# davidfang00/opticalflowdiffusion

Measured on AMD Instinct MI355X. Metric: UNet denoise steps/sec @ 2x436x1024 flow, bs=16, higher is better.
Workload: dtype bf16

## Files before the change

opticalflowdiffusion_amd/csrc/la_fused.hip:

```cpp
#include <cstdlib>
#include <type_traits>
#include "blocks.h"
#include "la_common.h"

namespace ofd {

template <int C>
struct XRaw {
    u32x4 v[C / 16];
};

template <int C>
__device__ __forceinline__ void load_raw_x(const bf16_t* __restrict__ xrow, XRaw<C>& r, int half) {
#pragma unroll
    for (int s = 0; s < C / 16; ++s) r.v[s] = *(const u32x4*)(xrow + 16 * s + 8 * half);
}

template <int N16, class At>
__device__ __forceinline__ void la_stage(unsigned char* dst, const bf16_t* __restrict__ src, int tid, At at) {
    static_assert(N16 % (8 * 256) == 0, "whole turns of eight units per thread");
    for (int i0 = tid; i0 < N16; i0 += 8 * 256) {
        uint4 v[8];
#pragma unroll
        for (int k = 0; k < 8; ++k) v[k] = ((const uint4*)src)[at(i0 + k * 256)];
#pragma unroll
        for (int k = 0; k < 8; ++k) ((uint4*)dst)[i0 + k * 256] = v[k];
    }
}
template <int N16>
__device__ __forceinline__ void la_stage(unsigned char* dst, const bf16_t* __restrict__ src, int tid) {
    la_stage<N16>(dst, src, tid, [](int i) { return i; });
}

typedef __bf16 la_bf16x2 __attribute__((ext_vector_type(2)));
template <int C>
__device__ __forceinline__ void norm_stats(const XRaw<C>& r, float eps, float& rstd, float& off) {
    const la_bf16x2 one = __builtin_bit_cast(la_bf16x2, 0x3f803f80u);
    float s1 = 0.0f, s2 = 0.0f;
#pragma unroll
    for (int s = 0; s < C / 16; ++s)
#pragma unroll
        for (int j = 0; j < 4; ++j) {
            const la_bf16x2 w = __builtin_bit_cast(la_bf16x2, (uint32_t)r.v[s][j]);
            s1 = __builtin_amdgcn_fdot2_f32_bf16(w, one, s1, false);
            s2 = __builtin_amdgcn_fdot2_f32_bf16(w, w, s2, false);
        }
    s1 += __shfl_xor(s1, 32, 64);
    s2 += __shfl_xor(s2, 32, 64);
    const float mean = s1 * (1.0f / C);
    const float var = fmaxf(__builtin_fmaf(-mean, mean, s2 * (1.0f / C)), 0.0f);
    rstd = rsqrtf(var + eps);
    off = -mean * rstd;
}
template <int C>
__device__ __forceinline__ void norm_x(const XRaw<C>& r, float eps, bf16x8 (&xs)[C / 16]) {
    float rstd, off;
    norm_stats<C>(r, eps, rstd, off);
#pragma unroll
    for (int s = 0; s < C / 16; ++s)
#pragma unroll
        for (int j = 0; j < 4; ++j) {
            const uint32_t w = r.v[s][j];
            xs[s][2 * j] = (__bf16)__builtin_fmaf(bf2f((bf16_t)(w & 0xffffu)), rstd, off);
            xs[s][2 * j + 1] = (__bf16)__builtin_fmaf(bf2f((bf16_t)(w >> 16)), rstd, off);
        }
}

template <int C>
__device__ __forceinline__ void norm_x_gain(const XRaw<C>& r, float eps, const float* __restrict__ g, int half, bf16x8 (&xs)[C / 16]) {
    float rstd, off;
    norm_stats<C>(r, eps, rstd, off);
#pragma unroll
    for (int s = 0; s < C / 16; ++s) {
        const float4 g0 = *(const float4*)(g + 16 * s + 8 * half), g1 = *(const float4*)(g + 16 * s + 8 * half + 4);
        const float gg[8] = {g0.x, g0.y, g0.z, g0.w, g1.x, g1.y, g1.z, g1.w};
#pragma unroll
        for (int j = 0; j < 4; ++j) {
            const uint32_t w = r.v[s][j];
            xs[s][2 * j] = (__bf16)(__builtin_fmaf(bf2f((bf16_t)(w & 0xffffu)), rstd, off) * gg[2 * j]);
            xs[s][2 * j + 1] = (__bf16)(__builtin_fmaf(bf2f((bf16_t)(w >> 16)), rstd, off) * gg[2 * j + 1]);
        }
    }
}

constexpr int LA_PART_PITCH = 64 + 32 * 36;
__device__ __forceinline__ void la_store_part(float* lds, float* __restrict__ o, float m, float l, const f32x16& ctxT, int tid, int wave, int l31,
                                              int half) {
    float* mine = lds + wave * LA_PART_PITCH;
    const float l_tot = l + __shfl_xor(l, 32, 64);
    if (half == 0) {
        mine[l31] = m;
        mine[32 + l31] = l_tot;
    }
#pragma unroll
    for (int g = 0; g < 4; ++g)
        *(float4*)(mine + 64 + l31 * 36 + 8 * g + 4 * half) = make_float4(ctxT[4 * g], ctxT[4 * g + 1], ctxT[4 * g + 2], ctxT[4 * g + 3]);
    __syncthreads();
    const int d = tid >> 3, e0 = (tid & 7) * 4;
    float mw[4], M = -3.0e38f;
#pragma unroll
    for (int w = 0; w < 4; ++w) {
        mw[w] = lds[w * LA_PART_PITCH + d];
        M = fmaxf(M, mw[w]);
    }
    float4 a = make_float4(0.0f, 0.0f, 0.0f, 0.0f);
    float ls = 0.0f;
#pragma unroll
    for (int w = 0; w < 4; ++w) {
        const float wt = __expf(mw[w] - M);
        const float4 v = *(const float4*)(lds + w * LA_PART_PITCH + 64 + d * 36 + e0);
        a.x += v.x * wt;
        a.y += v.y * wt;
        a.z += v.z * wt;
        a.w += v.w * wt;
        ls += lds[w * LA_PART_PITCH + 32 + d] * wt;
    }
    *(float4*)(o + 64 + d * 32 + e0) = a;
    if ((tid & 7) == 0) {
        o[d] = M;
        o[32 + d] = ls;
    }
    __syncthreads();
}

template <int NH>
__device__ __forceinline__ void ctx_state_init(f32x16 (&ctxT)[NH], float (&m)[NH], float (&l)[NH]) {
#pragma unroll
    for (int hd = 0; hd < NH; ++hd) {
        m[hd] = -3.0e38f;
        l[hd] = 0.0f;
#pragma unroll
        for (int r = 0; r < 16; ++r) ctxT[hd][r] = 0.0f;
    }
}
__device__ __forceinline__ f32x16 ctx_mask_rows(f32x16 ka, int tile, int n, int half) {
    if (tile * 32 + 32 > n) {
#pragma unroll
        for (int r = 0; r < 16; ++r)
            if (tile * 32 + acc_row(r, half) >= n) ka[r] = -3.0e38f;
    }
    return ka;
}
__device__ __forceinline__ float ctx_tile_max(const f32x16& ka) {
    float mt = -3.0e38f;
#pragma unroll
    for (int r = 0; r < 16; ++r) mt = fmaxf(mt, ka[r]);
    return fmaxf(mt, __shfl_xor(mt, 32, 64));
}
__device__ __forceinline__ void ctx_update(f32x16& ctxT, const f32x16& va, const f32x16& p) {
#pragma unroll
    for (int s2 = 0; s2 < 2; ++s2) ctxT = __builtin_amdgcn_mfma_f32_32x32x16_bf16(acc_frag(va, s2), acc_frag(p, s2), ctxT, 0, 0, 0);
}

template <int C, bool TRAIN, int HPW = 4>
__global__ void __launch_bounds__(256, C >= 256 ? 1 : 2) la_ctx_fused_kernel(const bf16_t* __restrict__ x, const bf16_t* __restrict__ wkv,
                                                           float* __restrict__ partial, int n, float eps, float defer,
                                                           const float* __restrict__ g, bf16_t* __restrict__ xn_out, bf16_t* __restrict__ qkv_out) {
    extern __shared__ __attribute__((aligned(16))) unsigned char smem[];
    static_assert(HPW == 4 || (HPW == 2 && !TRAIN), "the training form writes all four heads' k | v");
    constexpr int KS = C / 16, WR = 64 * HPW;
    const int tid = threadIdx.x, lane = tid & 63, wave = tid >> 6, l31 = lane & 31, half = lane >> 5;
    const int h0 = HPW == 4 ? 0 : blockIdx.z * HPW;
    if constexpr (C < 256) {
        for (int i = tid; i < (C / 8) * 256; i += 256) ((uint4*)smem)[i] = ((const uint4*)wkv)[i];
    } else {
        la_stage<(C / 8) * WR>(smem, wkv, tid, [&](int i) {
            const int r = i % WR, kv = r / (32 * HPW);
            return (i / WR) * 256 + kv * 128 + h0 * 32 + (r - kv * 32 * HPW);
        });
    }
    float* s_g = (float*)(smem + (C / 8) * WR * 16);
    if constexpr (TRAIN)
        for (int i = tid; i < C; i += 256) s_g[i] = g[i];
    __syncthreads();
    const int b = blockIdx.y, wave_id = blockIdx.x * 4 + wave, nw = gridDim.x * 4, ntiles = (n + 31) / 32;

    f32x16 ctxT[HPW];
    float m[HPW], l[HPW];
    ctx_state_init<HPW>(ctxT, m, l);
    const bf16_t* xb = x + (size_t)b * n * C;
    XRaw<C> raw_next;
    load_raw_x<C>(xb + (size_t)min(wave_id * 32 + l31, n - 1) * C, raw_next, half);
    for (int tile = wave_id; tile < ntiles; tile += nw) {
        asm volatile("" ::: "memory");
        const XRaw<C> raw = raw_next;
        load_raw_x<C>(xb + (size_t)min((tile + nw) * 32 + l31, n - 1) * C, raw_next, half);
        bf16x8 xs[KS];
        const int pix = tile * 32 + l31;
        if constexpr (TRAIN) {
            norm_x_gain<C>(raw, eps, s_g, half, xs);
            if (pix < n) {
                bf16_t* xrow = xn_out + ((size_t)b * n + pix) * C;
#pragma unroll
                for (int s = 0; s < KS; ++s) *(bf16x8*)(xrow + 16 * s + 8 * half) = xs[s];
            }
        } else {
            norm_x<C>(raw, eps, xs);
        }
        if constexpr (TRAIN) {
            bf16_t* qrow = qkv_out + ((size_t)b * n + min(pix, n - 1)) * 384 + 128;
#pragma unroll
            for (int blk = 0; blk < 8; ++blk) {
                f32x16 t;
#pragma unroll
                for (int r = 0; r < 16; ++r) t[r] = 0.0f;
#pragma unroll
                for (int s = 0; s < KS; ++s)
                    t = __builtin_amdgcn_mfma_f32_32x32x16_bf16(*(const bf16x8*)(smem + ((size_t)(2 * s + half) * 256 + blk * 32 + l31) * 16), xs[s], t, 0, 0, 0);
                store_acc_rows(t, qrow + blk * 32, half, pix < n);
            }
        }
#pragma unroll
        for (int hd = 0; hd < HPW; ++hd) {
            f32x16 ka, va;
#pragma unroll
            for (int r = 0; r < 16; ++r) { ka[r] = 0.0f; va[r] = 0.0f; }
#pragma unroll
            for (int s = 0; s < KS; ++s) {
                const bf16x8 wk = *(const bf16x8*)(smem + ((size_t)(2 * s + half) * WR + hd * 32 + l31) * 16);
                const bf16x8 wv = *(const bf16x8*)(smem + ((size_t)(2 * s + half) * WR + 32 * HPW + hd * 32 + l31) * 16);
                ka = __builtin_amdgcn_mfma_f32_32x32x16_bf16(xs[s], wk, ka, 0, 0, 0);
                va = __builtin_amdgcn_mfma_f32_32x32x16_bf16(xs[s], wv, va, 0, 0, 0);
            }
            if constexpr (TRAIN) {
#pragma unroll
                for (int r = 0; r < 16; ++r) ka[r] = bf2f(f2bf(ka[r]));
            }
            ka = ctx_mask_rows(ka, tile, n, half);
            const float mt = ctx_tile_max(ka);
            const bool move = mt > m[hd] + defer;
            if (__builtin_amdgcn_ballot_w64(move)) {
                const float m_new = move ? mt : m[hd];
                const float f = __expf(m[hd] - m_new);
                m[hd] = m_new;
                l[hd] *= f;
#pragma unroll
                for (int r = 0; r < 16; ++r) ctxT[hd][r] *= f;
            }
            float ps = 0.0f;
            const float m2 = m[hd] * LA_LOG2E;
#pragma unroll
            for (int r = 0; r < 16; ++r) {
                const float p = __builtin_amdgcn_exp2f(__builtin_fmaf(ka[r], LA_LOG2E, -m2));
                ka[r] = p;
                ps += p;
            }
            l[hd] += ps;
            ctx_update(ctxT[hd], va, ka);
            if constexpr (TRAIN) {
#pragma unroll
                for (int r = 0; r < 16; ++r) ka[r] -= (float)(__bf16)ka[r];
                ctx_update(ctxT[hd], va, ka);
            }
        }
    }
    __syncthreads();
#pragma unroll
    for (int hd = 0; hd < HPW; ++hd)
        la_store_part((float*)smem, partial + ((size_t)(b * 4 + h0 + hd) * gridDim.x + blockIdx.x) * 1088, m[hd], l[hd], ctxT[hd], tid, wave, l31, half);
}

__global__ void __launch_bounds__(256, 2) la_ctx_stored_kernel(const bf16_t* __restrict__ qkv, float* __restrict__ partial, int n) {
    const int tid = threadIdx.x, lane = tid & 63, wave = tid >> 6, l31 = lane & 31, half = lane >> 5;
    const int b = blockIdx.y, wave_id = blockIdx.x * 4 + wave, nw = gridDim.x * 4, ntiles = (n + 31) / 32;
    bf16x8 ident[2];
#pragma unroll
    for (int s2 = 0; s2 < 2; ++s2)
#pragma unroll
        for (int j = 0; j < 8; ++j) ident[s2][j] = (__bf16)((16 * s2 + 8 * half + j == l31) ? 1.0f : 0.0f);
    f32x16 ctxT[4];
    float m[4], l[4];
    ctx_state_init(ctxT, m, l);
    const bf16_t* qb = qkv + (size_t)b * n * 384;
    for (int tile = wave_id; tile < ntiles; tile += nw) {
        u32x4 kr[8], vr[8];
        {
            const bf16_t* row = qb + (size_t)min(tile * 32 + l31, n - 1) * 384 + 128 + 8 * half;
#pragma unroll
            for (int i = 0; i < 8; ++i) kr[i] = *(const u32x4*)(row + 16 * i);
#pragma unroll
            for (int i = 0; i < 8; ++i) vr[i] = *(const u32x4*)(row + 128 + 16 * i);
        }
#pragma unroll
        for (int hd = 0; hd < 4; ++hd) {
            f32x16 ka, va;
#pragma unroll
            for (int r = 0; r < 16; ++r) { ka[r] = 0.0f; va[r] = 0.0f; }
#pragma unroll
            for (int s2 = 0; s2 < 2; ++s2) {
                ka = __builtin_amdgcn_mfma_f32_32x32x16_bf16(__builtin_bit_cast(bf16x8, kr[hd * 2 + s2]), ident[s2], ka, 0, 0, 0);
                va = __builtin_amdgcn_mfma_f32_32x32x16_bf16(__builtin_bit_cast(bf16x8, vr[hd * 2 + s2]), ident[s2], va, 0, 0, 0);
            }
            ka = ctx_mask_rows(ka, tile, n, half);
            const float mt = ctx_tile_max(ka);
            const float m_new = fmaxf(m[hd], mt);
            const float f = __expf(m[hd] - m_new);
            m[hd] = m_new;
            float ps = 0.0f;
            const float m2 = m_new * LA_LOG2E;
#pragma unroll
            for (int r = 0; r < 16; ++r) {
                const float p = bf2f(f2bf(__builtin_amdgcn_exp2f(__builtin_fmaf(ka[r], LA_LOG2E, -m2))));
                ka[r] = p;
                ps += p;
            }
            l[hd] = l[hd] * f + ps;
#pragma unroll
            for (int r = 0; r < 16; ++r) ctxT[hd][r] *= f;
            ctx_update(ctxT[hd], va, ka);
        }
    }
    __shared__ __attribute__((aligned(16))) float part_s[4 * LA_PART_PITCH];
#pragma unroll
    for (int hd = 0; hd < 4; ++hd)
        la_store_part(part_s, partial + ((size_t)(b * 4 + hd) * gridDim.x + blockIdx.x) * 1088, m[hd], l[hd], ctxT[hd], tid, wave, l31, half);
}

int launch_la_ctx_stored(const bf16_t* qkv, float* partial, int B, int n, hipStream_t s) {
    const int gx = la_fused_blocks(n, B);
    la_ctx_stored_kernel<<<dim3(gx, B), 256, 0, s>>>(qkv, partial, n);
    return gx;
}

constexpr int LA_MAX_PARTS = 256;
template <class Out>
__global__ void __launch_bounds__(256) la_ctx_combine_kernel(const float* __restrict__ partial, Out* __restrict__ out, int nparts, float inv_n,
                                                             float* __restrict__ ml_out) {
    constexpr bool FRAG = std::is_same<Out, bf16_t>::value;
    __shared__ float red[8][32], M[32], Linv[32], w_s[LA_MAX_PARTS][32];
    const int tid = threadIdx.x, bh = blockIdx.x, dd = tid & 31, grp = tid >> 5;
    const float* base = partial + (size_t)bh * nparts * 1088;
    float mx = -3.0e38f;
    for (int c0 = grp; c0 < nparts; c0 += 32) {
        float t[4];
#pragma unroll
        for (int k = 0; k < 4; ++k) t[k] = base[(size_t)min(c0 + 8 * k, nparts - 1) * 1088 + dd];
#pragma unroll
        for (int k = 0; k < 4; ++k) mx = fmaxf(mx, t[k]);
    }
    red[grp][dd] = mx;
    __syncthreads();
    if (tid < 32) {
        float m = red[0][tid];
#pragma unroll
        for (int g = 1; g < 8; ++g) m = fmaxf(m, red[g][tid]);
        M[tid] = m;
    }
    __syncthreads();
    const bool use_ws = nparts <= LA_MAX_PARTS;
    float l = 0.0f;
    for (int c0 = grp; c0 < nparts; c0 += 32) {
        float tm[4], tl[4];
#pragma unroll
        for (int k = 0; k < 4; ++k) {
            const size_t o = (size_t)min(c0 + 8 * k, nparts - 1) * 1088;
            tm[k] = base[o + dd];
            tl[k] = base[o + 32 + dd];
        }
#pragma unroll
        for (int k = 0; k < 4; ++k)
            if (c0 + 8 * k < nparts) {
                const float w = __expf(tm[k] - M[dd]);
                if (use_ws) w_s[c0 + 8 * k][dd] = w;
                l += tl[k] * w;
            }
    }
    __syncthreads();
    red[grp][dd] = l;
    __syncthreads();
    if (tid < 32) {
        float t = red[0][tid];
#pragma unroll
        for (int g = 1; g < 8; ++g) t += red[g][tid];
        Linv[tid] = 1.0f / t;
        if (!FRAG && ml_out && blockIdx.y == 0) {
            ml_out[(size_t)bh * 64 + tid] = M[tid];
            ml_out[(size_t)bh * 64 + 32 + tid] = 1.0f / t;
        }
    }
    __syncthreads();
    const int i = blockIdx.y * 256 + tid;
    int d, e;
    if constexpr (FRAG) {
        const int j = i & 7, lane = (i >> 3) & 63, s2 = i >> 9;
        d = 16 * s2 + 8 * (j >> 2) + 4 * (lane >> 5) + (j & 3);
        e = lane & 31;
    } else {
        d = i >> 5;
        e = i & 31;
    }
    float a = 0.0f;
    for (int c0 = 0; c0 < nparts; c0 += 8) {
        float v[8];
#pragma unroll
        for (int k = 0; k < 8; ++k) v[k] = base[(size_t)min(c0 + k, nparts - 1) * 1088 + 64 + d * 32 + e];
        if (use_ws) {
#pragma unroll
            for (int k = 0; k < 8; ++k)
                if (c0 + k < nparts) a += v[k] * w_s[c0 + k][d];
        } else {
            float mc[8];
#pragma unroll
            for (int k = 0; k < 8; ++k) mc[k] = base[(size_t)min(c0 + k, nparts - 1) * 1088 + d];
#pragma unroll
            for (int k = 0; k < 8; ++k)
                if (c0 + k < nparts) a += v[k] * __expf(mc[k] - M[d]);
        }
    }
    const float c = a * Linv[d] * inv_n;
    if constexpr (FRAG) out[(size_t)bh * 1024 + i] = f2bf(c);
    else out[(size_t)bh * 1024 + i] = c;
}
void launch_la_ctx_combine(const float* partial, float* ctx, int B, int nparts, float inv_n, float* ml_out, hipStream_t s) {
    la_ctx_combine_kernel<<<dim3(B * 4, 4), 256, 0, s>>>(partial, ctx, nparts, inv_n, ml_out);
}

template <int C, bool TRAIN>
__device__ __forceinline__ f32x16 la_head_out(const bf16x8 (&xs)[C / 16], const unsigned char* s_wq, const unsigned char* s_cf, int hd, float scale,
                                              int lane) {
    const int l31 = lane & 31, half = lane >> 5;
    f32x16 qa;
#pragma unroll
    for (int r = 0; r < 16; ++r) qa[r] = 0.0f;
#pragma unroll
    for (int s = 0; s < C / 16; ++s) {
        const bf16x8 wf = *(const bf16x8*)(s_wq + ((size_t)(2 * s + half) * 128 + hd * 32 + l31) * 16);
        qa = __builtin_amdgcn_mfma_f32_32x32x16_bf16(wf, xs[s], qa, 0, 0, 0);
    }
    if constexpr (TRAIN) {
#pragma unroll
        for (int r = 0; r < 16; ++r) qa[r] = bf2f(f2bf(qa[r]));
    }
    const float k = scale / softmax_d(qa, 32);
#pragma unroll
    for (int r = 0; r < 16; ++r) qa[r] *= k;
    f32x16 oa;
#pragma unroll
    for (int r = 0; r < 16; ++r) oa[r] = 0.0f;
#pragma unroll
    for (int s2 = 0; s2 < 2; ++s2) {
        const bf16x8 cf = *(const bf16x8*)(s_cf + ((size_t)(hd * 2 + s2) * 64 + lane) * 16);
        oa = __builtin_amdgcn_mfma_f32_32x32x16_bf16(cf, acc_frag(qa, s2), oa, 0, 0, 0);
    }
    return oa;
}
template <int C>
__device__ __forceinline__ void la_to_out(f32x16 (&acc_o)[C / 32], const bf16x8 of, const unsigned char* s_wo, int u, int l31, int half) {
#pragma unroll
    for (int rt = 0; rt < C / 32; ++rt) {
        const bf16x8 wf = *(const bf16x8*)(s_wo + ((size_t)(u * 2 + half) * C + rt * 32 + l31) * 16);
        acc_o[rt] = __builtin_amdgcn_mfma_f32_32x32x16_bf16(wf, of, acc_o[rt], 0, 0, 0);
    }
}
template <int C, bool TRAIN, class XRes>
__device__ __forceinline__ void la_out_tail(f32x16 (&acc_o)[C / 32], XRes xres, const float* s_bias, const float* s_g2, bf16_t* yrow, bf16_t* orow, bool ok,
                                            int half, float eps_post) {
    constexpr int RT = C / 32;
    float sum = 0.0f;
#pragma unroll
    for (int rt = 0; rt < RT; ++rt)
#pragma unroll
        for (int g = 0; g < 4; ++g) {
            const float4 bv = *(const float4*)(s_bias + rt * 32 + 8 * g + 4 * half);
            acc_o[rt][4 * g] += bv.x; acc_o[rt][4 * g + 1] += bv.y; acc_o[rt][4 * g + 2] += bv.z; acc_o[rt][4 * g + 3] += bv.w;
            if constexpr (TRAIN) {
#pragma unroll
                for (int k = 0; k < 4; ++k) acc_o[rt][4 * g + k] = bf2f(f2bf(acc_o[rt][4 * g + k]));
            }
            sum += (acc_o[rt][4 * g] + acc_o[rt][4 * g + 1]) + (acc_o[rt][4 * g + 2] + acc_o[rt][4 * g + 3]);
        }
    if constexpr (TRAIN) {
#pragma unroll
        for (int rt = 0; rt < RT; ++rt) store_acc_rows(acc_o[rt], orow + rt * 32, half, ok);
    }
    sum += __shfl_xor(sum, 32, 64);
    const float mean = sum * (1.0f / C);
    float q = 0.0f;
#pragma unroll
    for (int rt = 0; rt < RT; ++rt)
#pragma unroll
        for (int r = 0; r < 16; ++r) { acc_o[rt][r] -= mean; q += acc_o[rt][r] * acc_o[rt][r]; }
    q += __shfl_xor(q, 32, 64);
    const float rstd = rsqrtf(q * (1.0f / C) + eps_post);
#pragma unroll
    for (int rt = 0; rt < RT; ++rt)
#pragma unroll
        for (int g = 0; g < 4; g += 2) {
            const u32x4 xw = xres(rt * 2 + (g >> 1));
            const uint4 xv = make_uint4(xw[0], xw[1], xw[2], xw[3]);
            const auto sx = __builtin_amdgcn_permlane32_swap(xv.x, xv.z, false, false);
            const auto sy = __builtin_amdgcn_permlane32_swap(xv.y, xv.w, false, false);
            const unsigned xq[2][2] = {{sx[0], sy[0]}, {sx[1], sy[1]}};
            uint2 qo[2];
#pragma unroll
            for (int k = 0; k < 2; ++k) {
                const int c0 = rt * 32 + 8 * (g + k) + 4 * half;
                const float4 gv = *(const float4*)(s_g2 + c0);
                const float o0 = acc_o[rt][4 * (g + k)] * rstd * gv.x + bf2f((bf16_t)(xq[k][0] & 0xffffu));
                const float o1 = acc_o[rt][4 * (g + k) + 1] * rstd * gv.y + bf2f((bf16_t)(xq[k][0] >> 16));
                const float o2 = acc_o[rt][4 * (g + k) + 2] * rstd * gv.z + bf2f((bf16_t)(xq[k][1] & 0xffffu));
                const float o3 = acc_o[rt][4 * (g + k) + 3] * rstd * gv.w + bf2f((bf16_t)(xq[k][1] >> 16));
                qo[k] = pack_quad(o0, o1, o2, o3);
            }
            store_quad_pair(yrow + rt * 32 + 8 * g, qo[0], qo[1], half, ok);
        }
}

template <int C, bool TRAIN>
__global__ void __launch_bounds__(256, C == 64 ? 4 : C == 128 ? 2 : 1) la_out_fused_kernel(const bf16_t* __restrict__ x, const bf16_t* __restrict__ wq,
                                                           const bf16_t* __restrict__ woutp, const bf16_t* __restrict__ ctxfrag,
                                                           const float* __restrict__ bias, const float* __restrict__ g2,
                                                           bf16_t* __restrict__ y, int n, float eps_pre, float eps_post, float scale,
                                                           const float* __restrict__ g, bf16_t* __restrict__ o2_out) {
    extern __shared__ __attribute__((aligned(16))) unsigned char smem[];
    constexpr int KS = C / 16, RT = C / 32;
    constexpr int WQ_B = (C / 8) * 128 * 16, WO_B = 16 * C * 16, CF_B = 4 * 2 * 64 * 16;
    unsigned char* s_wq = smem;
    unsigned char* s_wo = smem + WQ_B;
    unsigned char* s_cf = s_wo + WO_B;
    float* s_bias = (float*)(s_cf + CF_B);
    float* s_g2 = s_bias + C;
    float* s_g = s_g2 + C;
    const int tid = threadIdx.x, lane = tid & 63, wave = tid >> 6, l31 = lane & 31, half = lane >> 5;
    const int b = blockIdx.y;
    if constexpr (TRAIN)
        for (int i = tid; i < C; i += 256) s_g[i] = g[i];
    if constexpr (C < 256) {
        for (int i = tid; i < WQ_B / 16; i += 256) ((uint4*)s_wq)[i] = ((const uint4*)wq)[i];
        for (int i = tid; i < WO_B / 16; i += 256) ((uint4*)s_wo)[i] = ((const uint4*)woutp)[i];
    } else {
        la_stage<WQ_B / 16>(s_wq, wq, tid);
        la_stage<WO_B / 16>(s_wo, woutp, tid);
    }
    for (int i = tid; i < CF_B / 16; i += 256) ((uint4*)s_cf)[i] = ((const uint4*)(ctxfrag + (size_t)b * 4096))[i];
    for (int i = tid; i < C; i += 256) { s_bias[i] = bias[i]; s_g2[i] = g2[i]; }
    __syncthreads();
    const int wave_id = blockIdx.x * 4 + wave, nw = gridDim.x * 4, ntiles = (n + 31) / 32;

    const bf16_t* xb = x + (size_t)b * n * C;
    XRaw<C> raw_next;
    load_raw_x<C>(xb + (size_t)min(wave_id * 32 + l31, n - 1) * C, raw_next, half);
    for (int tile = wave_id; tile < ntiles; tile += nw) {
        asm volatile("" ::: "memory");
        const int pix = tile * 32 + l31;
        const size_t row = (size_t)b * n + min(pix, n - 1);
        const XRaw<C> raw = raw_next;
        load_raw_x<C>(xb + (size_t)min((tile + nw) * 32 + l31, n - 1) * C, raw_next, half);
        bf16x8 xs[KS];
        if constexpr (TRAIN) norm_x_gain<C>(raw, eps_pre, s_g, half, xs);
        else norm_x<C>(raw, eps_pre, xs);
        f32x16 acc_o[RT];
#pragma unroll
        for (int rt = 0; rt < RT; ++rt)
#pragma unroll
            for (int r = 0; r < 16; ++r) acc_o[rt][r] = 0.0f;
#pragma unroll
        for (int hd = 0; hd < 4; ++hd) {
            const f32x16 oa = la_head_out<C, TRAIN>(xs, s_wq, s_cf, hd, scale, lane);
#pragma unroll
            for (int s2 = 0; s2 < 2; ++s2) la_to_out<C>(acc_o, acc_frag(oa, s2), s_wo, hd * 2 + s2, l31, half);
        }
        la_out_tail<C, TRAIN>(acc_o, [&](int s) { return raw.v[s]; }, s_bias, s_g2, y + row * C, TRAIN ? o2_out + row * C : nullptr, pix < n, half, eps_post);
    }
}

template <int C>
__global__ void __launch_bounds__(256, 1) la_heads_kernel(const bf16_t* __restrict__ x, const bf16_t* __restrict__ wq, const bf16_t* __restrict__ ctxfrag,
                                                          bf16_t* __restrict__ y, int n, float eps_pre, float scale) {
    extern __shared__ __attribute__((aligned(16))) unsigned char smem[];
    constexpr int WQ_B = (C / 8) * 128 * 16, CF_B = 4 * 2 * 64 * 16;
    unsigned char* s_wq = smem;
    unsigned char* s_cf = smem + WQ_B;
    const int tid = threadIdx.x, lane = tid & 63, wave = tid >> 6, l31 = lane & 31, half = lane >> 5;
    const int b = blockIdx.y;
    la_stage<WQ_B / 16>(s_wq, wq, tid);
    for (int i = tid; i < CF_B / 16; i += 256) ((uint4*)s_cf)[i] = ((const uint4*)(ctxfrag + (size_t)b * 4096))[i];
    __syncthreads();
    const int wave_id = blockIdx.x * 4 + wave, nw = gridDim.x * 4, ntiles = (n + 31) / 32;
    const bf16_t* xb = x + (size_t)b * n * C;
    XRaw<C> raw_next;
    load_raw_x<C>(xb + (size_t)min(wave_id * 32 + l31, n - 1) * C, raw_next, half);
    for (int tile = wave_id; tile < ntiles; tile += nw) {
        asm volatile("" ::: "memory");
        const int pix = tile * 32 + l31;
        const XRaw<C> raw = raw_next;
        load_raw_x<C>(xb + (size_t)min((tile + nw) * 32 + l31, n - 1) * C, raw_next, half);
        bf16x8 xs[C / 16];
        norm_x<C>(raw, eps_pre, xs);
        bf16_t* arow = y + ((size_t)b * n + min(pix, n - 1)) * C + 8 * half;
#pragma unroll
        for (int hd = 0; hd < 4; ++hd) {
            const f32x16 oa = la_head_out<C, false>(xs, s_wq, s_cf, hd, scale, lane);
#pragma unroll
            for (int s2 = 0; s2 < 2; ++s2)
                if (pix < n) *(bf16x8*)(arow + (hd * 2 + s2) * 16) = acc_frag(oa, s2);
        }
    }
}

template <int C>
__global__ void __launch_bounds__(256, 1) la_tail_kernel(const bf16_t* __restrict__ x, const bf16_t* __restrict__ woutp, const float* __restrict__ bias,
                                                         const float* __restrict__ g2, bf16_t* y, int n, float eps_post) {
    extern __shared__ __attribute__((aligned(16))) unsigned char smem[];
    constexpr int RT = C / 32, WO_B = 16 * C * 16;
    unsigned char* s_wo = smem;
    float* s_bias = (float*)(smem + WO_B);
    float* s_g2 = s_bias + C;
    const int tid = threadIdx.x, lane = tid & 63, wave = tid >> 6, l31 = lane & 31, half = lane >> 5;
    const int b = blockIdx.y;
    la_stage<WO_B / 16>(s_wo, woutp, tid);
    for (int i = tid; i < C; i += 256) { s_bias[i] = bias[i]; s_g2[i] = g2[i]; }
    __syncthreads();
    const int wave_id = blockIdx.x * 4 + wave, nw = gridDim.x * 4, ntiles = (n + 31) / 32;
    const bf16_t* xb = x + (size_t)b * n * C;
    bf16_t* yb = y + (size_t)b * n * C;
    bf16x8 of_next[8];
    {
        const bf16_t* arow = yb + (size_t)min(wave_id * 32 + l31, n - 1) * C + 8 * half;
#pragma unroll
        for (int u = 0; u < 8; ++u) of_next[u] = *(const bf16x8*)(arow + u * 16);
    }
    for (int tile = wave_id; tile < ntiles; tile += nw) {
        asm volatile("" ::: "memory");
        const int pix = tile * 32 + l31;
        const size_t pid = min(pix, n - 1);
        bf16x8 of[8];
#pragma unroll
        for (int u = 0; u < 8; ++u) of[u] = of_next[u];
        {
            const bf16_t* arow = yb + (size_t)min((tile + nw) * 32 + l31, n - 1) * C + 8 * half;
#pragma unroll
            for (int u = 0; u < 8; ++u) of_next[u] = *(const bf16x8*)(arow + u * 16);
        }
        f32x16 acc_o[RT];
#pragma unroll
        for (int rt = 0; rt < RT; ++rt)
#pragma unroll
            for (int r = 0; r < 16; ++r) acc_o[rt][r] = 0.0f;
#pragma unroll
        for (int u = 0; u < 8; ++u) la_to_out<C>(acc_o, of[u], s_wo, u, l31, half);
        const bf16_t* xrow = xb + pid * C + 8 * half;
        la_out_tail<C, false>(acc_o, [&](int s) { return *(const u32x4*)(xrow + 16 * s); }, s_bias, s_g2, yb + pid * C, nullptr, pix < n, half, eps_post);
    }
}

__global__ void __launch_bounds__(256) la_weight_prep_kernel(const float* __restrict__ wqkv, const float* __restrict__ g, const float* __restrict__ wout,
                                                             bf16_t* __restrict__ wq, bf16_t* __restrict__ wkv, bf16_t* __restrict__ woutp, int C) {
    const int total = 512 * C;
    for (int i = blockIdx.x * blockDim.x + threadIdx.x; i < total; i += gridDim.x * blockDim.x) {
        if (i < 128 * C) {
            const int j = i & 7, o = (i >> 3) & 127, c8 = i >> 10, c = c8 * 8 + j;
            wq[i] = f2bf(wqkv[(size_t)o * C + c] * (g ? g[c] : 1.0f));
        } else if (i < 384 * C) {
            const int k = i - 128 * C;
            const int j = k & 7, o = (k >> 3) & 255, c8 = k >> 11, c = c8 * 8 + j;
            wkv[k] = f2bf(wqkv[(size_t)(128 + o) * C + c] * (g ? g[c] : 1.0f));
        } else if (woutp) {
            const int k = i - 384 * C;
            const int j = k & 7, c = (k >> 3) % C, rest = (k >> 3) / C;
            const int hh = rest & 1, s2 = (rest >> 1) & 1, hd = rest >> 2;
            woutp[k] = f2bf(wout[(size_t)c * 128 + hd * 32 + 16 * s2 + 8 * (j >> 2) + 4 * hh + (j & 3)]);
        }
    }
}

constexpr float LA_DEFER = 5.545177f;
constexpr int LA_GX2_CAP = 128;
static int la_out_blocks(int n, int B, int C) {
    if (C >= 256) {
        const int gx2 = cdiv(cdiv(n, 32), 4), cap2 = 256 / B;
        return gx2 < cap2 ? gx2 : (cap2 < 1 ? 1 : cap2);
    }
    int gx2 = cdiv(cdiv(n, 32), 4 * 4);
    if (gx2 < 1) gx2 = 1;
    const int cap2 = (LA_GX2_CAP * B < 1024) ? 1024 / B : LA_GX2_CAP;
    if (gx2 > cap2) gx2 = cap2;
    return gx2;
}

template <int C>
static int launch_la(const bf16_t* x, const bf16_t* wq, const bf16_t* wkv, const bf16_t* woutp, const float* bias, const float* g2,
                     float* partial, bf16_t* ctxfrag, bf16_t* y, int B, int n, float eps_pre, float eps_post, hipStream_t s) {
    constexpr int HPW = C == 512 ? 2 : 4;
    constexpr bool SPLIT2 = C == 512;
    constexpr int LDS1 = (C / 8) * 64 * HPW * 16;
    constexpr int LDS2 = (C / 8) * 128 * 16 + 16 * C * 16 + 4 * 2 * 64 * 16 + 2 * C * 4;
    constexpr int LDS2H = (C / 8) * 128 * 16 + 4 * 2 * 64 * 16, LDS2T = 16 * C * 16 + 2 * C * 4;
    static_assert(LDS1 <= 160 * 1024 && (SPLIT2 ? LDS2H <= 160 * 1024 && LDS2T <= 160 * 1024 : LDS2 <= 160 * 1024), "the weights of a pass must fit the LDS");
    static bool attr = false;
    if (!attr) {
        OFD_HIP(hipFuncSetAttribute((const void*)la_ctx_fused_kernel<C, false, HPW>, hipFuncAttributeMaxDynamicSharedMemorySize, LDS1));
        if constexpr (SPLIT2) {
            OFD_HIP(hipFuncSetAttribute((const void*)la_heads_kernel<C>, hipFuncAttributeMaxDynamicSharedMemorySize, LDS2H));
            OFD_HIP(hipFuncSetAttribute((const void*)la_tail_kernel<C>, hipFuncAttributeMaxDynamicSharedMemorySize, LDS2T));
        } else {
            OFD_HIP(hipFuncSetAttribute((const void*)la_out_fused_kernel<C, false>, hipFuncAttributeMaxDynamicSharedMemorySize, LDS2));
        }
        attr = true;
    }
    const int gx = la_fused_blocks(n, B, C), gx2 = la_out_blocks(n, B, C);
    la_ctx_fused_kernel<C, false, HPW><<<dim3(gx, B, 4 / HPW), 256, LDS1, s>>>(x, wkv, partial, n, eps_pre, LA_DEFER, nullptr, nullptr, nullptr);
    la_ctx_combine_kernel<<<dim3(B * 4, 4), 256, 0, s>>>(partial, ctxfrag, gx, 1.0f / (float)n, nullptr);
    if constexpr (SPLIT2) {
        la_heads_kernel<C><<<dim3(gx2, B), 256, LDS2H, s>>>(x, wq, ctxfrag, y, n, eps_pre, LA_SCALE);
        la_tail_kernel<C><<<dim3(gx2, B), 256, LDS2T, s>>>(x, woutp, bias, g2, y, n, eps_post);
    } else {
        la_out_fused_kernel<C, false><<<dim3(gx2, B), 256, LDS2, s>>>(x, wq, woutp, ctxfrag, bias, g2, y, n, eps_pre, eps_post, LA_SCALE, nullptr, nullptr);
    }
    OFD_LAUNCH_CHECK();
    return OFD_OK;
}

int k_linear_attention_fused_train(const bf16_t* x, const bf16_t* wq, const bf16_t* wkv, const bf16_t* woutp, const float* bias, const float* g_pre,
                                   const float* g2, float* partial, bf16_t* ctxfrag, float* ctx, float* ml, bf16_t* xn, bf16_t* qkv, bf16_t* o2,
                                   bf16_t* y, int B, int n, int C, float eps_pre, float eps_post, hipStream_t s) {
    if (C != 64) { set_error("linear_attention_fused_train: C=%d unsupported", C); return OFD_ERR_ARG; }
    constexpr int LDS1 = (64 / 8) * 256 * 16 + 64 * 4;
    constexpr int LDS2 = (64 / 8) * 128 * 16 + 16 * 64 * 16 + 4 * 2 * 64 * 16 + 3 * 64 * 4;
    static bool attr = false;
    if (!attr) {
        OFD_HIP(hipFuncSetAttribute((const void*)la_ctx_fused_kernel<64, true>, hipFuncAttributeMaxDynamicSharedMemorySize, LDS1));
        OFD_HIP(hipFuncSetAttribute((const void*)la_out_fused_kernel<64, true>, hipFuncAttributeMaxDynamicSharedMemorySize, LDS2));
        attr = true;
    }
    const int gx = la_fused_blocks(n, B);
    la_ctx_fused_kernel<64, true><<<dim3(gx, B), 256, LDS1, s>>>(x, wkv, partial, n, eps_pre, LA_DEFER, g_pre, xn, qkv);
    la_ctx_combine_kernel<<<dim3(B * 4, 4), 256, 0, s>>>(partial, ctxfrag, gx, 1.0f / (float)n, nullptr);
    launch_la_ctx_combine(partial, ctx, B, gx, 1.0f / (float)n, ml, s);
    la_out_fused_kernel<64, true><<<dim3(la_out_blocks(n, B, 64), B), 256, LDS2, s>>>(x, wq, woutp, ctxfrag, bias, g2, y, n, eps_pre, eps_post, LA_SCALE, g_pre, o2);
    OFD_LAUNCH_CHECK();
    return OFD_OK;
}

int la_fused_blocks(int n, int B, int C) {
    constexpr int total = 256;
    int gx = cdiv(cdiv(n, 32), 8);
    int cap = total / (B < 1 ? 1 : B);
    if (C >= 256) cap = (cap < 32 ? 32 : cap) / (C / 256);
    else if (cap < 64) cap = 64;
    if (cap < 1) cap = 1;
    if (gx < 1) gx = 1;
    if (gx > cap) gx = cap;
    return gx;
}

int k_la_weight_prep(const float* wqkv, const float* g, const float* wout, bf16_t* wq, bf16_t* wkv, bf16_t* woutp, int C, hipStream_t s) {
    la_weight_prep_kernel<<<cdiv((woutp ? 512 : 384) * C, 256), 256, 0, s>>>(wqkv, g, wout, wq, wkv, woutp, C);
    OFD_LAUNCH_CHECK();
    return OFD_OK;
}

int k_linear_attention_fused(const bf16_t* x, const bf16_t* wq, const bf16_t* wkv, const bf16_t* woutp, const float* bias, const float* g2,
                             float* partial, bf16_t* ctxfrag, bf16_t* y, int B, int n, int C, float eps_pre, float eps_post, hipStream_t s) {
    if (C == 64) return launch_la<64>(x, wq, wkv, woutp, bias, g2, partial, ctxfrag, y, B, n, eps_pre, eps_post, s);
    if (C == 128) return launch_la<128>(x, wq, wkv, woutp, bias, g2, partial, ctxfrag, y, B, n, eps_pre, eps_post, s);
    if (C == 256) return launch_la<256>(x, wq, wkv, woutp, bias, g2, partial, ctxfrag, y, B, n, eps_pre, eps_post, s);
    if (C == 512) return launch_la<512>(x, wq, wkv, woutp, bias, g2, partial, ctxfrag, y, B, n, eps_pre, eps_post, s);
    set_error("linear_attention_fused: C=%d unsupported", C);
    return OFD_ERR_ARG;
}

}
```

Before: 35.69.

## Use 512-thread blocks for wide-channel linear attention and drop register prefetch

For C>=256 the linear-attention context, fused-output and heads kernels now launch 512 threads (8 waves) per block instead of 256. The double-buffered raw-x register prefetch is removed or deferred in those paths to cut register pressure. Residual x is re-read from global memory in the tail, and grid sizes are rebalanced, with the ctx grid capped at 16 blocks when B>=8. This trades prefetch latency hiding and partial-reduction parallelism for more waves per CU sharing one weight copy in LDS.

```diff
diff --git a/opticalflowdiffusion_amd/csrc/la_fused.hip b/opticalflowdiffusion_amd/csrc/la_fused.hip
--- a/opticalflowdiffusion_amd/csrc/la_fused.hip
+++ b/opticalflowdiffusion_amd/csrc/la_fused.hip
@@ -16,20 +16,21 @@
     for (int s = 0; s < C / 16; ++s) r.v[s] = *(const u32x4*)(xrow + 16 * s + 8 * half);
 }
 
-template <int N16, class At>
+template <int N16, int NT, class At>
 __device__ __forceinline__ void la_stage(unsigned char* dst, const bf16_t* __restrict__ src, int tid, At at) {
-    static_assert(N16 % (8 * 256) == 0, "whole turns of eight units per thread");
-    for (int i0 = tid; i0 < N16; i0 += 8 * 256) {
-        uint4 v[8];
-#pragma unroll
-        for (int k = 0; k < 8; ++k) v[k] = ((const uint4*)src)[at(i0 + k * 256)];
-#pragma unroll
-        for (int k = 0; k < 8; ++k) ((uint4*)dst)[i0 + k * 256] = v[k];
-    }
-}
-template <int N16>
+    constexpr int K = N16 % (8 * NT) == 0 ? 8 : 4;
+    static_assert(N16 % (K * NT) == 0, "whole turns of K units per thread");
+    for (int i0 = tid; i0 < N16; i0 += K * NT) {
+        uint4 v[K];
+#pragma unroll
+        for (int k = 0; k < K; ++k) v[k] = ((const uint4*)src)[at(i0 + k * NT)];
+#pragma unroll
+        for (int k = 0; k < K; ++k) ((uint4*)dst)[i0 + k * NT] = v[k];
+    }
+}
+template <int N16, int NT>
 __device__ __forceinline__ void la_stage(unsigned char* dst, const bf16_t* __restrict__ src, int tid) {
-    la_stage<N16>(dst, src, tid, [](int i) { return i; });
+    la_stage<N16, NT>(dst, src, tid, [](int i) { return i; });
 }
 
 typedef __bf16 la_bf16x2 __attribute__((ext_vector_type(2)));
@@ -84,6 +85,7 @@
 }
 
 constexpr int LA_PART_PITCH = 64 + 32 * 36;
+template <int NW = 4>
 __device__ __forceinline__ void la_store_part(float* lds, float* __restrict__ o, float m, float l, const f32x16& ctxT, int tid, int wave, int l31,
                                               int half) {
     float* mine = lds + wave * LA_PART_PITCH;
@@ -96,29 +98,31 @@
     for (int g = 0; g < 4; ++g)
         *(float4*)(mine + 64 + l31 * 36 + 8 * g + 4 * half) = make_float4(ctxT[4 * g], ctxT[4 * g + 1], ctxT[4 * g + 2], ctxT[4 * g + 3]);
     __syncthreads();
-    const int d = tid >> 3, e0 = (tid & 7) * 4;
-    float mw[4], M = -3.0e38f;
-#pragma unroll
-    for (int w = 0; w < 4; ++w) {
-        mw[w] = lds[w * LA_PART_PITCH + d];
-        M = fmaxf(M, mw[w]);
-    }
-    float4 a = make_float4(0.0f, 0.0f, 0.0f, 0.0f);
-    float ls = 0.0f;
-#pragma unroll
-    for (int w = 0; w < 4; ++w) {
-        const float wt = __expf(mw[w] - M);
-        const float4 v = *(const float4*)(lds + w * LA_PART_PITCH + 64 + d * 36 + e0);
-        a.x += v.x * wt;
-        a.y += v.y * wt;
-        a.z += v.z * wt;
-        a.w += v.w * wt;
-        ls += lds[w * LA_PART_PITCH + 32 + d] * wt;
-    }
-    *(float4*)(o + 64 + d * 32 + e0) = a;
-    if ((tid & 7) == 0) {
-        o[d] = M;
-        o[32 + d] = ls;
+    if (NW == 4 || tid < 256) {
+        const int d = tid >> 3, e0 = (tid & 7) * 4;
+        float mw[NW], M = -3.0e38f;
+#pragma unroll
+        for (int w = 0; w < NW; ++w) {
+            mw[w] = lds[w * LA_PART_PITCH + d];
+            M = fmaxf(M, mw[w]);
+        }
+        float4 a = make_float4(0.0f, 0.0f, 0.0f, 0.0f);
+        float ls = 0.0f;
+#pragma unroll
+        for (int w = 0; w < NW; ++w) {
+            const float wt = __expf(mw[w] - M);
+            const float4 v = *(const float4*)(lds + w * LA_PART_PITCH + 64 + d * 36 + e0);
+            a.x += v.x * wt;
+            a.y += v.y * wt;
+            a.z += v.z * wt;
+            a.w += v.w * wt;
+            ls += lds[w * LA_PART_PITCH + 32 + d] * wt;
+        }
+        *(float4*)(o + 64 + d * 32 + e0) = a;
+        if ((tid & 7) == 0) {
+            o[d] = M;
+            o[32 + d] = ls;
+        }
     }
     __syncthreads();
 }
@@ -152,39 +156,44 @@
     for (int s2 = 0; s2 < 2; ++s2) ctxT = __builtin_amdgcn_mfma_f32_32x32x16_bf16(acc_frag(va, s2), acc_frag(p, s2), ctxT, 0, 0, 0);
 }
 
+constexpr int la_threads(int C) { return C >= 256 ? 512 : 256; }
 template <int C, bool TRAIN, int HPW = 4>
-__global__ void __launch_bounds__(256, C >= 256 ? 1 : 2) la_ctx_fused_kernel(const bf16_t* __restrict__ x, const bf16_t* __restrict__ wkv,
+__global__ void __launch_bounds__(la_threads(C), C >= 256 ? 1 : 2) la_ctx_fused_kernel(const bf16_t* __restrict__ x, const bf16_t* __restrict__ wkv,
                                                            float* __restrict__ partial, int n, float eps, float defer,
                                                            const float* __restrict__ g, bf16_t* __restrict__ xn_out, bf16_t* __restrict__ qkv_out) {
     extern __shared__ __attribute__((aligned(16))) unsigned char smem[];
     static_assert(HPW == 4 || (HPW == 2 && !TRAIN), "the training form writes all four heads' k | v");
     constexpr int KS = C / 16, WR = 64 * HPW;
+    constexpr int NT = la_threads(C), NW = NT / 64;
+    constexpr bool PREFETCH = C < 256;
     const int tid = threadIdx.x, lane = tid & 63, wave = tid >> 6, l31 = lane & 31, half = lane >> 5;
     const int h0 = HPW == 4 ? 0 : blockIdx.z * HPW;
-    if constexpr (C < 256) {
-        for (int i = tid; i < (C / 8) * 256; i += 256) ((uint4*)smem)[i] = ((const uint4*)wkv)[i];
-    } else {
-        la_stage<(C / 8) * WR>(smem, wkv, tid, [&](int i) {
-            const int r = i % WR, kv = r / (32 * HPW);
-            return (i / WR) * 256 + kv * 128 + h0 * 32 + (r - kv * 32 * HPW);
-        });
-    }
+    la_stage<(C / 8) * WR, NT>(smem, wkv, tid, [&](int i) {
+        if constexpr (HPW == 4) return i;
+        const int r = i % WR, kv = r / (32 * HPW);
+        return (i / WR) * 256 + kv * 128 + h0 * 32 + (r - kv * 32 * HPW);
+    });
     float* s_g = (float*)(smem + (C / 8) * WR * 16);
     if constexpr (TRAIN)
-        for (int i = tid; i < C; i += 256) s_g[i] = g[i];
-    __syncthreads();
-    const int b = blockIdx.y, wave_id = blockIdx.x * 4 + wave, nw = gridDim.x * 4, ntiles = (n + 31) / 32;
+        for (int i = tid; i < C; i += NT) s_g[i] = g[i];
+    __syncthreads();
+    const int b = blockIdx.y, wave_id = blockIdx.x * NW + wave, nw = gridDim.x * NW, ntiles = (n + 31) / 32;
 
     f32x16 ctxT[HPW];
     float m[HPW], l[HPW];
     ctx_state_init<HPW>(ctxT, m, l);
     const bf16_t* xb = x + (size_t)b * n * C;
     XRaw<C> raw_next;
-    load_raw_x<C>(xb + (size_t)min(wave_id * 32 + l31, n - 1) * C, raw_next, half);
+    if constexpr (PREFETCH) load_raw_x<C>(xb + (size_t)min(wave_id * 32 + l31, n - 1) * C, raw_next, half);
     for (int tile = wave_id; tile < ntiles; tile += nw) {
         asm volatile("" ::: "memory");
-        const XRaw<C> raw = raw_next;
-        load_raw_x<C>(xb + (size_t)min((tile + nw) * 32 + l31, n - 1) * C, raw_next, half);
+        XRaw<C> raw;
+        if constexpr (PREFETCH) {
+            raw = raw_next;
+            load_raw_x<C>(xb + (size_t)min((tile + nw) * 32 + l31, n - 1) * C, raw_next, half);
+        } else {
+            load_raw_x<C>(xb + (size_t)min(tile * 32 + l31, n - 1) * C, raw, half);
+        }
         bf16x8 xs[KS];
         const int pix = tile * 32 + l31;
         if constexpr (TRAIN) {
@@ -257,7 +266,7 @@
     __syncthreads();
 #pragma unroll
     for (int hd = 0; hd < HPW; ++hd)
-        la_store_part((float*)smem, partial + ((size_t)(b * 4 + h0 + hd) * gridDim.x + blockIdx.x) * 1088, m[hd], l[hd], ctxT[hd], tid, wave, l31, half);
+        la_store_part<NW>((float*)smem, partial + ((size_t)(b * 4 + h0 + hd) * gridDim.x + blockIdx.x) * 1088, m[hd], l[hd], ctxT[hd], tid, wave, l31, half);
 }
 
 __global__ void __launch_bounds__(256, 2) la_ctx_stored_kernel(const bf16_t* __restrict__ qkv, float* __restrict__ partial, int n) {
@@ -507,7 +516,7 @@
 }
 
 template <int C, bool TRAIN>
-__global__ void __launch_bounds__(256, C == 64 ? 4 : C == 128 ? 2 : 1) la_out_fused_kernel(const bf16_t* __restrict__ x, const bf16_t* __restrict__ wq,
+__global__ void __launch_bounds__(la_threads(C), C == 64 ? 4 : C == 128 ? 2 : 1) la_out_fused_kernel(const bf16_t* __restrict__ x, const bf16_t* __restrict__ wq,
                                                            const bf16_t* __restrict__ woutp, const bf16_t* __restrict__ ctxfrag,
                                                            const float* __restrict__ bias, const float* __restrict__ g2,
                                                            bf16_t* __restrict__ y, int n, float eps_pre, float eps_post, float scale,
@@ -523,19 +532,16 @@
     float* s_g = s_g2 + C;
     const int tid = threadIdx.x, lane = tid & 63, wave = tid >> 6, l31 = lane & 31, half = lane >> 5;
     const int b = blockIdx.y;
+    constexpr int NT = la_threads(C), NW = NT / 64;
+    constexpr bool WIDE = C >= 256;
     if constexpr (TRAIN)
-        for (int i = tid; i < C; i += 256) s_g[i] = g[i];
-    if constexpr (C < 256) {
-        for (int i = tid; i < WQ_B / 16; i += 256) ((uint4*)s_wq)[i] = ((const uint4*)wq)[i];
-        for (int i = tid; i < WO_B / 16; i += 256) ((uint4*)s_wo)[i] = ((const uint4*)woutp)[i];
-    } else {
-        la_stage<WQ_B / 16>(s_wq, wq, tid);
-        la_stage<WO_B / 16>(s_wo, woutp, tid);
-    }
-    for (int i = tid; i < CF_B / 16; i += 256) ((uint4*)s_cf)[i] = ((const uint4*)(ctxfrag + (size_t)b * 4096))[i];
-    for (int i = tid; i < C; i += 256) { s_bias[i] = bias[i]; s_g2[i] = g2[i]; }
-    __syncthreads();
-    const int wave_id = blockIdx.x * 4 + wave, nw = gridDim.x * 4, ntiles = (n + 31) / 32;
+        for (int i = tid; i < C; i += NT) s_g[i] = g[i];
+    la_stage<WQ_B / 16, NT>(s_wq, wq, tid);
+    la_stage<WO_B / 16, NT>(s_wo, woutp, tid);
+    for (int i = tid; i < CF_B / 16; i += NT) ((uint4*)s_cf)[i] = ((const uint4*)(ctxfrag + (size_t)b * 4096))[i];
+    for (int i = tid; i < C; i += NT) { s_bias[i] = bias[i]; s_g2[i] = g2[i]; }
+    __syncthreads();
+    const int wave_id = blockIdx.x * NW + wave, nw = gridDim.x * NW, ntiles = (n + 31) / 32;
 
     const bf16_t* xb = x + (size_t)b * n * C;
     XRaw<C> raw_next;
@@ -545,7 +551,7 @@
         const int pix = tile * 32 + l31;
         const size_t row = (size_t)b * n + min(pix, n - 1);
         const XRaw<C> raw = raw_next;
-        load_raw_x<C>(xb + (size_t)min((tile + nw) * 32 + l31, n - 1) * C, raw_next, half);
+        if constexpr (!WIDE) load_raw_x<C>(xb + (size_t)min((tile + nw) * 32 + l31, n - 1) * C, raw_next, half);
         bf16x8 xs[KS];
         if constexpr (TRAIN) norm_x_gain<C>(raw, eps_pre, s_g, half, xs);
         else norm_x<C>(raw, eps_pre, xs);
@@ -560,12 +566,18 @@
 #pragma unroll
             for (int s2 = 0; s2 < 2; ++s2) la_to_out<C>(acc_o, acc_frag(oa, s2), s_wo, hd * 2 + s2, l31, half);
         }
-        la_out_tail<C, TRAIN>(acc_o, [&](int s) { return raw.v[s]; }, s_bias, s_g2, y + row * C, TRAIN ? o2_out + row * C : nullptr, pix < n, half, eps_post);
-    }
-}
-
-template <int C>
-__global__ void __launch_bounds__(256, 1) la_heads_kernel(const bf16_t* __restrict__ x, const bf16_t* __restrict__ wq, const bf16_t* __restrict__ ctxfrag,
+        if constexpr (WIDE) {
+            load_raw_x<C>(xb + (size_t)min((tile + nw) * 32 + l31, n - 1) * C, raw_next, half);
+            const bf16_t* xrow = x + row * C + 8 * half;
+            la_out_tail<C, TRAIN>(acc_o, [&](int s) { return *(const u32x4*)(xrow + 16 * s); }, s_bias, s_g2, y + row * C, nullptr, pix < n, half, eps_post);
+        } else {
+            la_out_tail<C, TRAIN>(acc_o, [&](int s) { return raw.v[s]; }, s_bias, s_g2, y + row * C, TRAIN ? o2_out + row * C : nullptr, pix < n, half, eps_post);
+        }
+    }
+}
+
+template <int C>
+__global__ void __launch_bounds__(512, 1) la_heads_kernel(const bf16_t* __restrict__ x, const bf16_t* __restrict__ wq, const bf16_t* __restrict__ ctxfrag,
                                                           bf16_t* __restrict__ y, int n, float eps_pre, float scale) {
     extern __shared__ __attribute__((aligned(16))) unsigned char smem[];
     constexpr int WQ_B = (C / 8) * 128 * 16, CF_B = 4 * 2 * 64 * 16;
@@ -573,18 +585,16 @@
     unsigned char* s_cf = smem + WQ_B;
     const int tid = threadIdx.x, lane = tid & 63, wave = tid >> 6, l31 = lane & 31, half = lane >> 5;
     const int b = blockIdx.y;
-    la_stage<WQ_B / 16>(s_wq, wq, tid);
-    for (int i = tid; i < CF_B / 16; i += 256) ((uint4*)s_cf)[i] = ((const uint4*)(ctxfrag + (size_t)b * 4096))[i];
-    __syncthreads();
-    const int wave_id = blockIdx.x * 4 + wave, nw = gridDim.x * 4, ntiles = (n + 31) / 32;
+    la_stage<WQ_B / 16, 512>(s_wq, wq, tid);
+    for (int i = tid; i < CF_B / 16; i += 512) ((uint4*)s_cf)[i] = ((const uint4*)(ctxfrag + (size_t)b * 4096))[i];
+    __syncthreads();
+    const int wave_id = blockIdx.x * 8 + wave, nw = gridDim.x * 8, ntiles = (n + 31) / 32;
     const bf16_t* xb = x + (size_t)b * n * C;
-    XRaw<C> raw_next;
-    load_raw_x<C>(xb + (size_t)min(wave_id * 32 + l31, n - 1) * C, raw_next, half);
     for (int tile = wave_id; tile < ntiles; tile += nw) {
         asm volatile("" ::: "memory");
         const int pix = tile * 32 + l31;
-        const XRaw<C> raw = raw_next;
-        load_raw_x<C>(xb + (size_t)min((tile + nw) * 32 + l31, n - 1) * C, raw_next, half);
+        XRaw<C> raw;
+        load_raw_x<C>(xb + (size_t)min(pix, n - 1) * C, raw, half);
         bf16x8 xs[C / 16];
         norm_x<C>(raw, eps_pre, xs);
         bf16_t* arow = y + ((size_t)b * n + min(pix, n - 1)) * C + 8 * half;
@@ -608,7 +618,7 @@
     float* s_g2 = s_bias + C;
     const int tid = threadIdx.x, lane = tid & 63, wave = tid >> 6, l31 = lane & 31, half = lane >> 5;
     const int b = blockIdx.y;
-    la_stage<WO_B / 16>(s_wo, woutp, tid);
+    la_stage<WO_B / 16, 256>(s_wo, woutp, tid);
     for (int i = tid; i < C; i += 256) { s_bias[i] = bias[i]; s_g2[i] = g2[i]; }
     __syncthreads();
     const int wave_id = blockIdx.x * 4 + wave, nw = gridDim.x * 4, ntiles = (n + 31) / 32;
@@ -666,9 +676,9 @@
 
 constexpr float LA_DEFER = 5.545177f;
 constexpr int LA_GX2_CAP = 128;
-static int la_out_blocks(int n, int B, int C) {
+static int la_out_blocks(int n, int B, int C, int waves = 8) {
     if (C >= 256) {
-        const int gx2 = cdiv(cdiv(n, 32), 4), cap2 = 256 / B;
+        const int gx2 = cdiv(cdiv(n, 32), waves), cap2 = 256 / B;
         return gx2 < cap2 ? gx2 : (cap2 < 1 ? 1 : cap2);
     }
     int gx2 = cdiv(cdiv(n, 32), 4 * 4);
@@ -699,13 +709,13 @@
         attr = true;
     }
     const int gx = la_fused_blocks(n, B, C), gx2 = la_out_blocks(n, B, C);
-    la_ctx_fused_kernel<C, false, HPW><<<dim3(gx, B, 4 / HPW), 256, LDS1, s>>>(x, wkv, partial, n, eps_pre, LA_DEFER, nullptr, nullptr, nullptr);
+    la_ctx_fused_kernel<C, false, HPW><<<dim3(gx, B, 4 / HPW), la_threads(C), LDS1, s>>>(x, wkv, partial, n, eps_pre, LA_DEFER, nullptr, nullptr, nullptr);
     la_ctx_combine_kernel<<<dim3(B * 4, 4), 256, 0, s>>>(partial, ctxfrag, gx, 1.0f / (float)n, nullptr);
     if constexpr (SPLIT2) {
-        la_heads_kernel<C><<<dim3(gx2, B), 256, LDS2H, s>>>(x, wq, ctxfrag, y, n, eps_pre, LA_SCALE);
-        la_tail_kernel<C><<<dim3(gx2, B), 256, LDS2T, s>>>(x, woutp, bias, g2, y, n, eps_post);
+        la_heads_kernel<C><<<dim3(gx2, B), 512, LDS2H, s>>>(x, wq, ctxfrag, y, n, eps_pre, LA_SCALE);
+        la_tail_kernel<C><<<dim3(la_out_blocks(n, B, C, 4), B), 256, LDS2T, s>>>(x, woutp, bias, g2, y, n, eps_post);
     } else {
-        la_out_fused_kernel<C, false><<<dim3(gx2, B), 256, LDS2, s>>>(x, wq, woutp, ctxfrag, bias, g2, y, n, eps_pre, eps_post, LA_SCALE, nullptr, nullptr);
+        la_out_fused_kernel<C, false><<<dim3(gx2, B), la_threads(C), LDS2, s>>>(x, wq, woutp, ctxfrag, bias, g2, y, n, eps_pre, eps_post, LA_SCALE, nullptr, nullptr);
     }
     OFD_LAUNCH_CHECK();
     return OFD_OK;
@@ -736,7 +746,7 @@
     constexpr int total = 256;
     int gx = cdiv(cdiv(n, 32), 8);
     int cap = total / (B < 1 ? 1 : B);
-    if (C >= 256) cap = (cap < 32 ? 32 : cap) / (C / 256);
+    if (C >= 256) cap = (B >= 8 ? 16 : cap) / (C / 256);
     else if (cap < 64) cap = 64;
     if (cap < 1) cap = 1;
     if (gx < 1) gx = 1;
```

Measured after the change: 35.83, median of 3. About the same (+0.4%).
